# jackdent/cs265-lsm-tree

Hardware: AMD Instinct MI355X
Metric: Bloom build+probe Gkeys/s device-resident; achieved HBM GB/s vs roofline (higher is better)
Workload: dtype int32 keys, u64 hash arithmetic

## Files before the change

cs265-lsm-tree_amd/csrc/bloom_pass1.h:

```cpp
#pragma once

#include "bloom_prims.h"

namespace bloomhip {

namespace {


constexpr int kPrioSort = 0, kPrioScatter = 1, kPrioHash = 2, kPrioYoung = 3;
constexpr int pass1_prio_of(int mode, int level) { return level | mode << 2; }

template <int LAYOUT, int TB>
__device__ __forceinline__ void load_tile_keys(const KeySpan &ks, size_t tile, int tid,
                                               int32_t (&k)[kPartKPT]) {
    static_assert(kPartKPT == 8, "two int4 / four entry pairs per thread");
    const size_t i0 = tile * (size_t)(TB * kPartKPT) + (size_t)kPartKPT * tid;
    const bool full = (tile + 1) * (size_t)(TB * kPartKPT) <= ks.n;
    if constexpr (LAYOUT == KEYS_PACKED) {
        if (full) {
            const int4 *v = reinterpret_cast<const int4 *>(ks.base) + i0 / 4;
            const int4 a = v[0], b = v[1];
            k[0] = a.x; k[1] = a.y; k[2] = a.z; k[3] = a.w;
            k[4] = b.x; k[5] = b.y; k[6] = b.z; k[7] = b.w;
            return;
// ... 2 lines not shown
        if (full) {
            const int4 *v = reinterpret_cast<const int4 *>(ks.base) + i0 / 2;
            const int4 a = v[0], b = v[1], c = v[2], d = v[3];
            k[0] = a.x; k[1] = a.z; k[2] = b.x; k[3] = b.z;
            k[4] = c.x; k[5] = c.z; k[6] = d.x; k[7] = d.z;
            return;
        }
    }
#pragma unroll
    for (int j = 0; j < kPartKPT; j++) {
        const size_t i = i0 + j;
        k[j] = i < ks.n ? load_key<LAYOUT>(ks, i) : 0;
    }
}

__device__ __forceinline__ size_t part_tile(size_t k, size_t ntiles) {
    const size_t base = k * gridDim.x;
    if (base >= ntiles) return ntiles;
    const size_t nr = min((size_t)gridDim.x, ntiles - base);
    return blockIdx.x < nr ? base + xcd_remap(blockIdx.x, (unsigned)nr) : ntiles;
}

template <typename P>
__device__ __forceinline__ uint32_t seg_of(P p, const SegMap &sm) {
    return __umulhi((uint32_t)(p >> sm.shift), sm.magic);
}

constexpr uint32_t kBinShift = 19;

constexpr int kModFast = 0, kModWide = 1, kModP2 = 2, kModLadder = 3, kModLadder0 = 4;
constexpr int kModLadder0R = 5;

template <int MK, int MINW>
__device__ __forceinline__ void bin_entry(uint64_t raw, const ModParams &mp, const SegMap &sm,
                                          uint32_t &b, uint32_t &ent) {
    if constexpr (MK == kModWide) {
        const uint64_t p = mod_wide(raw, mp);
        b = seg_of(p, sm);
        ent = (uint32_t)p & kEntryMask;
    } else if constexpr (MK == kModLadder) {
        const uint32_t xl = (uint32_t)raw;
        const uint32_t a = mod_p2_hi(raw, mp);
        b = __builtin_amdgcn_ubfe(xl, sm.shift, sm.lad_u);
        const uint32_t ehi =
            (a << sm.lad_hb) + __builtin_amdgcn_ubfe(xl, sm.scaled_shift, sm.lad_hb);
        ent = (ehi << sm.shift) | __builtin_amdgcn_ubfe(xl, 0, sm.shift);
    } else if constexpr (MK == kModLadder0) {
        const uint32_t xl = (uint32_t)raw;
        if constexpr (MINW >= 6) {
            const uint32_t lo = __builtin_amdgcn_ubfe(xl, 0, sm.shift);
            b = __builtin_amdgcn_ubfe(xl, sm.shift, sm.lad_u);
            ent = lshl_or_s(mod_p2_hi(raw, mp), sm.shift, lo);
        } else {
            const uint32_t a = mod_p2_hi(raw, mp);
            b = __builtin_amdgcn_ubfe(xl, sm.shift, sm.lad_u);
            ent = (a << sm.shift) | __builtin_amdgcn_ubfe(xl, 0, sm.shift);
        }
    } else if constexpr (MK == kModLadder0R) {
        const uint32_t xl = (uint32_t)raw;
        if constexpr (MINW >= 6) {
            const uint32_t lo = __builtin_amdgcn_ubfe(xl, 0, sm.shift);
            b = __builtin_amdgcn_ubfe(xl, sm.shift, sm.lad_u);
            ent = lshl_or_s(mod_p2_hi24(raw, mp), sm.shift, lo);
        } else {
            const uint32_t a = mod_p2_hi24(raw, mp);
            b = __builtin_amdgcn_ubfe(xl, sm.shift, sm.lad_u);
            ent = (a << sm.shift) | __builtin_amdgcn_ubfe(xl, 0, sm.shift);
        }
    } else if constexpr (MK == kModP2) {
        const uint32_t xl = (uint32_t)raw;
        const uint32_t r = mod_p2_hi(raw, mp);
        const uint32_t q = (r << sm.p2_hi_shift) |
                           __builtin_amdgcn_ubfe(xl, sm.shift, sm.p2_hi_shift);
        b = __umulhi(q, sm.magic);
        ent = xl & kEntryMask;
    } else {
        const uint32_t ru = mod_fast_scaled(raw, mp);
        b = __umulhi(ru >> sm.scaled_shift, sm.magic);
        ent = __builtin_amdgcn_ubfe(ru, mp.l, kEntryBits);
    }
}

template <int LAYOUT, bool SLOTS, bool COLS, int TB, int MK, int MAXB = 0, int MINW = 4,
          int ABL = 0, bool NT = false, bool DEFER = false, int PRIO = 0>
__global__ void __launch_bounds__(TB, MINW) k_part_bin(KeySpan ks, ModParams mp,
                                                       uint64_t *__restrict__ pos_out,
                                                       uint32_t *__restrict__ runs, SegMap sm,
                                                       size_t ntiles, uint16_t *__restrict__ slots) {
    constexpr int kTileKeys = TB * kPartKPT;
    constexpr int kTilePos = 3 * kTileKeys;
    constexpr int kMaxB = MAXB ? MAXB : TB >= 1024 ? (int)kPartMaxBinsBig : (int)kPartMaxBins;
    constexpr int kScanPer = (kMaxB + 1 + TB - 1) / TB;
    static_assert(4 * kTilePos <= (1 << 17) && kTilePos < (1 << 16) &&
                      ((uint64_t)(kMaxB - 1) << kBinShift) < (1ull << 32),
                  "packed rank fields (bin nbins, never incremented, may wrap to 0)");
    constexpr int kPrioLevel = PRIO & 3, kPrioMode = PRIO >> 2;
    static_assert(PRIO == 0 || (kPrioLevel > 0 && kPrioMode <= kPrioYoung), "PRIO = level | mode << 2");
    constexpr bool kFlips = PRIO != 0 && kPrioMode != kPrioYoung;
    constexpr int kPrioAtHist = !kFlips ? -1 : kPrioMode == kPrioHash ? kPrioLevel : 0;
    constexpr int kPrioAtRank = !kFlips || kPrioMode == kPrioScatter ? -1 : kPrioMode == kPrioSort ? kPrioLevel : 0;
    constexpr int kPrioAtScan = kFlips && kPrioMode == kPrioScatter ? kPrioLevel : -1;
    __shared__ __attribute__((aligned(16))) uint32_t s_sorted[kTilePos];
    __shared__ uint32_t s_hist[kMaxB + 1];
    __shared__ uint32_t s_wsum[TB / 64];

    const int tid = threadIdx.x;
    const int lane = tid & 63, wave = tid >> 6;
    const int nb = (int)sm.nbins;
    const int per = (nb + 1 + TB - 1) / TB;
    int32_t kcur[kPartKPT], knext[kPartKPT];

    constexpr int kVecs = kTileKeys / 2;
    constexpr int kStores = kVecs / TB;
    static_assert(kStores * TB == kVecs && kStores * 2 == kPartKPT, "whole vectors per thread");
    auto pack_store = [&](auto full_c, int r, size_t tile, int tile_keys) {
        constexpr bool FULL = decltype(full_c)::value;
        uint4 *dst = reinterpret_cast<uint4 *>(pos_out + tile * (size_t)kTileKeys) + r * TB + tid;
        const uint2 *src = reinterpret_cast<const uint2 *>(s_sorted + 6 * (r * TB + tid));
        const uint2 a = src[0], b = src[1], c = src[2];
        uint32_t e[6] = {a.x, a.y, b.x, b.y, c.x, c.y};
        if constexpr (!FULL) {
#pragma unroll
            for (int q = 0; q < 6; q++) e[q] = 6 * (r * TB + tid) + q < 3 * tile_keys ? e[q] & kEntryMask : 0u;
        }
        const uint4 v = pack_entries6(e);
        if constexpr (ABL == 0) {
            if constexpr (NT) nt_store16(dst, v);
            else *dst = v;
        } else {
            if (v.x == 0xFFFFFFFFu && v.y == 0xFFFFFFFFu) *dst = v;
        }
    };
    constexpr bool kPacks = ABL == 0 || ABL == 5;

    auto do_tile = [&](auto full_c, auto prev_c, size_t tile, size_t next, size_t prev) {
        constexpr bool FULL = decltype(full_c)::value;
        constexpr bool PREV = decltype(prev_c)::value && kPacks;
        const size_t tile0 = tile * kTileKeys;
        const int tile_keys = FULL ? (int)kTileKeys : (int)min((size_t)kTileKeys, ks.n - tile0);
        auto live = [&](int j) { return FULL || kPartKPT * tid + j < tile_keys; };
#pragma clang loop unroll(disable) vectorize(disable)
        for (int b = tid; b <= nb; b += TB) s_hist[b] = (uint32_t)b << kBinShift;
        lds_barrier_prio<kPrioAtHist>();

        uint32_t br[kPartKPT * 3];
        uint32_t ent[kPartKPT * 3];
#pragma unroll
        for (int j = 0; j < kPartKPT; j++) {
            if constexpr (PREV) {
                if (j & 1) pack_store(BoolC<true>{}, j / 2, prev, kTileKeys);
            }
            if (live(j)) {
                const int32_t k = kcur[j];
#pragma unroll
                for (int h = 0; h < 3; h++) {
                    const uint64_t raw = h == 0 ? raw_hash1(k) : h == 1 ? raw_hash2(k) : raw_hash3(k);
                    uint32_t b, e;
                    bin_entry<MK, MINW>(raw, mp, sm, b, e);
                    ent[3 * j + h] = e;
                    if constexpr (ABL == 1) br[3 * j + h] = b;
                    else br[3 * j + h] = atomicAdd(&s_hist[b], 4u);
                }
            } else {
#pragma unroll
                for (int h = 0; h < 3; h++) br[3 * j + h] = ent[3 * j + h] = 0;
            }
        }
        lds_barrier_prio<kPrioAtRank>();
        auto consume = [&]() {
            uint32_t x = 0;
#pragma unroll
            for (int q = 0; q < 3 * kPartKPT; q++) x ^= br[q] + ent[q];
            if (x == 0x9E3779B9u) reinterpret_cast<uint32_t *>(pos_out)[tile * kTileKeys + tid] = x;
        };
        if constexpr (ABL == 1 || ABL == 2) {
            if (next < ntiles) load_tile_keys<LAYOUT, TB>(ks, next, tid, knext);
            consume();
            return;
        }

        const bool scan_wave = wave * 64 * per <= nb;
        uint32_t local[kScanPer];
        uint32_t tsum = 0, incl = 0;
        if (scan_wave) {
#pragma unroll
            for (int q = 0; q < kScanPer; q++) {
                const int b = tid * per + q;
                local[q] = (q < per && b <= nb) ? s_hist[b] - ((uint32_t)b << kBinShift) : 0u;
                tsum += local[q];
            }
            incl = wave_incl_scan(tsum);
            if (lane == 63) s_wsum[wave] = incl;
        }
        lds_barrier();
        if (scan_wave) {
            uint32_t run = incl - tsum;
            for (int w = 0; w < wave; w++) run += s_wsum[w];
#pragma unroll
            for (int q = 0; q < kScanPer; q++) {
                const int b = tid * per + q;
                if (q < per && b <= nb) {
                    s_hist[b] = run - ((uint32_t)b << kBinShift);
                    const uint32_t pk = (run >> 2) | (((run + local[q]) >> 2) << 16);
                    if (b < nb) {
                        if constexpr (COLS) runs[(size_t)b * ntiles + tile] = pk;
                        else runs[tile * (size_t)nb + b] = pk;
                    }
                    run += local[q];
                }
            }
        }
        lds_barrier_prio<kPrioAtScan>();
        if (next < ntiles) load_tile_keys<LAYOUT, TB>(ks, next, tid, knext);
        if constexpr (ABL == 3) {
            consume();
            return;
        }

        const char *hist_b = reinterpret_cast<const char *>(s_hist);
        char *sorted_b = reinterpret_cast<char *>(s_sorted);
#pragma unroll
        for (int h = 0; h < 3; h++) {
            uint32_t slot[kPartKPT];
#pragma unroll
            for (int j = 0; j < kPartKPT; j++)
                slot[j] = *reinterpret_cast<const uint32_t *>(hist_b + (br[3 * j + h] >> 17)) +
                          br[3 * j + h];
#pragma unroll
            for (int j = 0; j < kPartKPT; j++)
                if (live(j)) *reinterpret_cast<uint32_t *>(sorted_b + slot[j]) = ent[3 * j + h];
            if constexpr (SLOTS) {
                uint16_t *sl = slots + (tile * 3 + h) * kTileKeys + kPartKPT * tid;
                if (FULL) {
                    uint32_t w[kPartKPT / 2];
#pragma unroll
                    for (int q = 0; q < kPartKPT / 2; q++)
                        w[q] = lshl_or(slot[2 * q + 1], 14, slot[2 * q] >> 2);
                    typedef uint32_t v4u __attribute__((ext_vector_type(4)));
                    const v4u wv = {w[0], w[1], w[2], w[3]};
                    __builtin_nontemporal_store(wv, reinterpret_cast<v4u *>(sl));
                } else {
#pragma unroll
                    for (int j = 0; j < kPartKPT; j++)
                        if (live(j)) sl[j] = (uint16_t)(slot[j] >> 2);
                }
            }
        }
        lds_barrier();
        if constexpr (ABL == 4) {
            if ((s_sorted[tid] ^ br[0]) == 0x9E3779B9u)
                reinterpret_cast<uint32_t *>(pos_out)[tile * kTileKeys + tid] = br[0];
            return;
        }
        if constexpr (!DEFER) {
#pragma unroll
            for (int r = 0; r < kStores; r++) pack_store(full_c, r, tile, tile_keys);
        }
    };
    auto write_out = [&](auto full_c, size_t tile) {
        if constexpr (DEFER && kPacks) {
            const int tile_keys = (int)min((size_t)kTileKeys, ks.n - tile * kTileKeys);
#pragma unroll
            for (int r = 0; r < kStores; r++) pack_store(full_c, r, tile, tile_keys);
        }
    };

    const size_t nfull = ks.n / kTileKeys;
    size_t tile = part_tile(0, ntiles);
    if (tile >= ntiles) return;
    if constexpr (PRIO != 0 && kPrioMode == kPrioYoung) {
        if (__builtin_amdgcn_readfirstlane(threadIdx.x) >= TB / 2) __builtin_amdgcn_s_setprio(kPrioLevel);
    }
    load_tile_keys<LAYOUT, TB>(ks, tile, tid, kcur);
    if constexpr (!DEFER) {
        for (size_t round = 0; tile < nfull; round++) {
            const size_t next = part_tile(round + 1, ntiles);
            do_tile(BoolC<true>{}, BoolC<false>{}, tile, next, tile);
#pragma unroll
            for (int j = 0; j < kPartKPT; j++) kcur[j] = knext[j];
            tile = next;
        }
        if (tile < ntiles) do_tile(BoolC<false>{}, BoolC<false>{}, tile, ntiles, tile);
    } else if (tile >= nfull) {
        do_tile(BoolC<false>{}, BoolC<false>{}, tile, ntiles, tile);
        write_out(BoolC<false>{}, tile);
    } else {
        size_t prev = tile;
        {
            const size_t next = part_tile(1, ntiles);
            do_tile(BoolC<true>{}, BoolC<false>{}, tile, next, tile);
#pragma unroll
            for (int j = 0; j < kPartKPT; j++) kcur[j] = knext[j];
            tile = next;
        }
        for (size_t round = 1; tile < nfull; round++) {
            const size_t next = part_tile(round + 1, ntiles);
            do_tile(BoolC<true>{}, BoolC<true>{}, tile, next, prev);
#pragma unroll
            for (int j = 0; j < kPartKPT; j++) kcur[j] = knext[j];
            prev = tile;
            tile = next;
        }
        if (tile < ntiles) {
            do_tile(BoolC<false>{}, BoolC<true>{}, tile, ntiles, prev);
            write_out(BoolC<false>{}, tile);
        } else {
            write_out(BoolC<true>{}, prev);
        }
    }
}

constexpr uint32_t kBinShift2 = 20;
constexpr int kSuperBlock = 1024;

template <int LAYOUT>
__device__ __forceinline__ void load_half_keys(const KeySpan &ks, size_t tile, int half, int tid,
                                               int32_t (&k)[kPartKPT]) {
    constexpr size_t kHalf = (size_t)kSuperBlock * kPartKPT;
    const size_t i0 = tile * kSuperTileKeys + half * kHalf + (size_t)kPartKPT * tid;
    const bool full = tile * kSuperTileKeys + (half + 1) * kHalf <= ks.n;
    if constexpr (LAYOUT == KEYS_PACKED) {
        if (full) {
            const int4 *v = reinterpret_cast<const int4 *>(ks.base) + i0 / 4;
            const int4 a = v[0], b = v[1];
            k[0] = a.x; k[1] = a.y; k[2] = a.z; k[3] = a.w;
            k[4] = b.x; k[5] = b.y; k[6] = b.z; k[7] = b.w;
            return;
        }
    } else if constexpr (LAYOUT == KEYS_ENTRY) {
        if (full) {
            const int4 *v = reinterpret_cast<const int4 *>(ks.base) + i0 / 2;
            const int4 a = v[0], b = v[1], c = v[2], d = v[3];
            k[0] = a.x; k[1] = a.z; k[2] = b.x; k[3] = b.z;
            k[4] = c.x; k[5] = c.z; k[6] = d.x; k[7] = d.z;
            return;
        }
    }
#pragma unroll
    for (int j = 0; j < kPartKPT; j++) {
        const size_t i = i0 + j;
        k[j] = i < ks.n ? load_key<LAYOUT>(ks, i) : 0;
    }
}

template <int LAYOUT, bool COLS, int MK, int MAXB, bool SLOTS = false>
__global__ void __launch_bounds__(kSuperBlock, 4) k_part_bin2(KeySpan ks, ModParams mp,
                                                              uint64_t *__restrict__ pos_out,
                                                              uint32_t *__restrict__ runs, SegMap sm,
                                                              size_t ntiles, uint16_t *__restrict__ slots) {
    constexpr int TB = kSuperBlock;
    constexpr int kHalfKeys = TB * kPartKPT;
    constexpr int kTileKeys = 2 * kHalfKeys;
    constexpr int kTilePos = 3 * kTileKeys;
    constexpr int kPhasePos = kTilePos / 2;
    constexpr uint32_t kPhaseBytes = 4u * kPhasePos;
    constexpr int kScanPer = (MAXB + 1 + TB - 1) / TB;
    constexpr int kPer = 3 * kPartKPT;
// ... 150 lines not shown
#pragma unroll
        for (int ph = 0; ph < 2; ph++) {
            const uint32_t base = ph * kPhaseBytes;
            uint2 w[kPartKPT];
#pragma unroll
            for (int j = 0; j < kPartKPT; j++) w[j] = stash[j * TB + tid];
#pragma unroll
            for (int j = 0; j < kPartKPT; j++) {
#pragma unroll
                for (int h = 0; h < 3; h++) {
                    const uint32_t la = brA[3 * j + h] - base;
                    if (la < kPhaseBytes) {
                        const uint32_t e = h == 0 ? w[j].x & kEntryMask
                                         : h == 1 ? __builtin_amdgcn_alignbit(w[j].y, w[j].x, 21) & kEntryMask
                                                  : w[j].y >> 10;
                        *reinterpret_cast<uint32_t *>(img_b + la) = e;
                    }
                }
            }
#pragma unroll
            for (int j = 0; j < kPartKPT; j++) {
#pragma unroll
                for (int h = 0; h < 3; h++) {
                    const uint32_t lb = brB[3 * j + h] - base;
                    if (lb < kPhaseBytes) {
                        const uint32_t lo = eB[2 * j], hi = eB[2 * j + 1];
                        const uint32_t e = h == 0 ? lo & kEntryMask
                                         : h == 1 ? __builtin_amdgcn_alignbit(hi, lo, 21) & kEntryMask
                                                  : hi >> 10;
                        *reinterpret_cast<uint32_t *>(img_b + lb) = e;
                    }
                }
            }
            lds_barrier();
#pragma unroll
            for (int r = 0; r < kStores; r++) {
                const uint2 *src = reinterpret_cast<const uint2 *>(img + 6 * (r * TB + tid));
                const uint2 a = src[0], b = src[1], c = src[2];
                uint32_t e[6] = {a.x, a.y, b.x, b.y, c.x, c.y};
                if constexpr (!FULL) {
#pragma unroll
                    for (int z = 0; z < 6; z++) e[z] &= kEntryMask;
                }
                dst[ph * kVecs + r * TB + tid] = pack_entries6(e);
            }
            if (ph == 0) lds_barrier();
        }
    };

    const size_t nfull = ks.n / kTileKeys;
    size_t tile = part_tile(0, ntiles);
    if (tile < ntiles) load_half_keys<LAYOUT>(ks, tile, 0, (int)threadIdx.x, kA);
    size_t round = 0;
    for (; tile < nfull; round++) {
        const size_t next = part_tile(round + 1, ntiles);
        do_tile(BoolC<true>{}, tile, next);
        tile = next;
    }
    if (tile < ntiles) do_tile(BoolC<false>{}, tile, ntiles);
}

constexpr size_t kColumnTableMaxBytes = 16u << 20;
constexpr int kTransposeTile = 64;
constexpr int kTransposeBlock = 256;

}

hipError_t launch_runs_transpose(const PartitionWorkspace &ws, hipStream_t stream);
bool runs_as_columns(const PartitionWorkspace &ws);

struct Pass1Kernel {
    bool super;
    int threads;
    int layout;
    bool slots;
    bool cols;
    int mk;
    int maxb;
    int wgs_per_cu;
    bool nt;
    bool defer;
    unsigned grid;
    int prio;
};
using Pass1Launch = bool(const Pass1Kernel &p, const KeySpan &ks, const ModParams &mp,
                         const PartitionWorkspace &ws, const SegMap &sm, uint16_t *slots,
                         hipStream_t stream);
Pass1Launch launch_bin_build512, launch_bin_build1024, launch_bin_probe512, launch_bin_probe1024,
    launch_bin_super, launch_bin_super_probe;

namespace {

constexpr int pass1_max_bins(bool super, int threads) {
    return super ? (int)kSuperMaxBins : threads >= 1024 ? (int)kPartMaxBinsBig : (int)kPartMaxBins;
}

constexpr bool pass1_takes_kind(bool super, bool slots, int mk) {
    if (super) return mk == kModP2 || mk == kModFast;
    return mk >= 0 && !(slots && (mk == kModLadder0 || mk == kModLadder0R));
}

constexpr int pass1_capacity(int threads, int layout, int mk, size_t nbins) {
    const int cap = pass1_max_bins(false, threads);
    if (layout == KEYS_STRIDED || mk == kModWide) return cap;
    if (threads >= 1024) return nbins <= 1023 ? 1023 : nbins <= 2047 ? 2047 : nbins <= 4095 ? 4095 : cap;
    return nbins <= 511 ? 511 : cap;
}

constexpr int pass1_wgs_per_cu(int threads, bool slots, int maxb) {
    return threads >= 1024 ? 1 : (!slots && maxb > 0 && maxb <= 511) ? 3 : 2;
}
constexpr int pass1_min_waves(int threads, int wgs) { return wgs * threads / 256; }
inline unsigned pass1_grid(size_t ntiles, int ncu, int wgs) {
    const size_t g = (size_t)ncu * wgs;
    return (unsigned)(ntiles < g ? ntiles : g);
}

constexpr bool pass1_defer(int threads, bool slots) { return threads >= 1024 && !slots; }

constexpr int pass1_prio(int threads, bool slots, int wgs_per_cu) {
    return threads == 512 && !slots && wgs_per_cu == 3 ? pass1_prio_of(kPrioHash, 1) : 0;
}

constexpr bool pass1_may_nt(int threads, bool slots, int maxb) {
    return !slots && threads >= 1024 && maxb == 1023;
}

inline bool p2_pass1(const ModParams &mp, const SegMap &sm) {
    return mp.fast && mp.p2 && mp.p2t >= kEntryBits && sm.shift <= mp.p2t && mp.p2t - sm.shift < 32;
}

inline int pass1_plan(const ModParams &mp, const PartitionWorkspace &ws, bool slots, SegMap *out) {
    SegMap sm = seg_map_of(ws);
    const bool wide = !mp.fast;
    if (!wide) {
        sm.scaled_shift = sm.shift + mp.l;
        if (sm.scaled_shift > 31) {
            sm.scaled_shift = 0;
            sm.magic = 0;
        }
    }
    int mk;
    if (ws.lad_u) {
        if (!mp.fast || !mp.p2 || sm.shift + sm.lad_u + sm.lad_hb != mp.p2t) return -1;
        sm.scaled_shift = sm.shift + sm.lad_u;
        mk = sm.lad_hb == 0 && !slots ? (ladder0_relabel(mp, ws) ? kModLadder0R : kModLadder0) : kModLadder;
    } else if (wide) {
        mk = kModWide;
    } else if (p2_pass1(mp, sm)) {
        sm.p2_hi_shift = mp.p2t - sm.shift;
        mk = kModP2;
    } else {
        mk = kModFast;
    }
    *out = sm;
    return mk;
}

inline bool choose_pass1_kernel(const KeySpan &ks, const ModParams &mp, const PartitionWorkspace &ws,
                                bool slots, int ncu, Pass1Kernel *out, SegMap *sm) {
    Pass1Kernel p{};
    p.super = tile_keys_of(ws) == kSuperTileKeys;
    p.threads = p.super ? kSuperBlock : tile_keys_of(ws) == 2 * kPartTileKeys ? 1024 : 512;
    p.slots = slots;
    if (ws.nbins > (size_t)pass1_max_bins(p.super, p.threads)) return false;
    p.mk = pass1_plan(mp, ws, slots, sm);
    if (p.mk < 0 || !pass1_takes_kind(p.super, slots, p.mk)) return false;
    p.layout = ks.layout == KEYS_PACKED ? KEYS_PACKED
               : ks.layout == KEYS_ENTRY && (reinterpret_cast<uintptr_t>(ks.base) & 15) == 0 ? KEYS_ENTRY
                                                                                               : KEYS_STRIDED;
    p.maxb = p.super ? (int)kSuperMaxBins : pass1_capacity(p.threads, p.layout, p.mk, ws.nbins);
    p.wgs_per_cu = p.super ? 1 : pass1_wgs_per_cu(p.threads, slots, p.maxb);
    p.defer = !p.super && pass1_defer(p.threads, slots);
    p.nt = !p.super && pass1_may_nt(p.threads, slots, p.maxb) &&
           ws.ntiles * (uint64_t)(p.threads * kPartKPT) * 8 > kInfinityCacheBytes;
    p.prio = p.super ? 0 : pass1_prio(p.threads, slots, p.wgs_per_cu);
    p.cols = runs_as_columns(ws);
    p.grid = pass1_grid(ws.ntiles, ncu, p.wgs_per_cu);
    *out = p;
    return true;
}

template <bool SLOTS, int TB>
bool launch_pass1_tile(const Pass1Kernel &p, const KeySpan &ks, const ModParams &mp,
                       const PartitionWorkspace &ws, const SegMap &sm, uint16_t *slots,
                       hipStream_t stream) {
    constexpr bool kDefer = pass1_defer(TB, SLOTS);
    if (p.super || p.threads != TB || p.slots != SLOTS || p.defer != kDefer) return false;
    uint32_t *runs = p.cols ? ws.run_starts : ws.run_rows;
    return on_value<kModFast, kModWide, kModP2, kModLadder, kModLadder0, kModLadder0R>(p.mk, [&](auto mk_c) {
        return on_value<KEYS_PACKED, KEYS_ENTRY, KEYS_STRIDED>(p.layout, [&](auto layout_c) {
            return on_value<511, 1023, 2047, 4095, pass1_max_bins(false, TB)>(p.maxb, [&](auto maxb_c) {
                constexpr int MK = decltype(mk_c)::value, L = decltype(layout_c)::value;
                constexpr int MAXB = decltype(maxb_c)::value;
                constexpr bool kHeld = pass1_takes_kind(false, SLOTS, MK) && pass1_capacity(TB, L, MK, MAXB) == MAXB;
                if constexpr (kHeld) {
                    constexpr int kWgs = pass1_wgs_per_cu(TB, SLOTS, MAXB);
                    constexpr int kMinW = pass1_min_waves(TB, kWgs);
                    constexpr bool kMayNT = pass1_may_nt(TB, SLOTS, MAXB);
                    constexpr int kPrio = pass1_prio(TB, SLOTS, kWgs);
                    if (p.wgs_per_cu != kWgs || (p.nt && !kMayNT) || p.prio != kPrio) return false;
                    auto go = [&](auto cols_c, auto nt_c) {
                        k_part_bin<L, SLOTS, decltype(cols_c)::value, TB, MK, MAXB, kMinW, 0,
                                   decltype(nt_c)::value, kDefer, kPrio>
                            <<<p.grid, TB, 0, stream>>>(ks, mp, ws.pos, runs, sm, ws.ntiles, slots);
                    };
                    if constexpr (kMayNT) {
                        if (p.nt) {
                            p.cols ? go(BoolC<true>{}, BoolC<true>{}) : go(BoolC<false>{}, BoolC<true>{});
                            return true;
                        }
                    }
                    p.cols ? go(BoolC<true>{}, BoolC<false>{}) : go(BoolC<false>{}, BoolC<false>{});
                    return true;
                } else {
                    return false;
                }
            });
        });
    });
}

template <bool SLOTS>
bool launch_pass1_super(const Pass1Kernel &p, const KeySpan &ks, const ModParams &mp,
                        const PartitionWorkspace &ws, const SegMap &sm, uint16_t *slots,
                        hipStream_t stream) {
    if (!p.super || p.slots != SLOTS) return false;
    uint32_t *runs = p.cols ? ws.run_starts : ws.run_rows;
    return on_value<kModP2, kModFast>(p.mk, [&](auto mk_c) {
        return on_value<KEYS_PACKED, KEYS_ENTRY, KEYS_STRIDED>(p.layout, [&](auto layout_c) {
            auto go = [&](auto cols_c) {
                k_part_bin2<decltype(layout_c)::value, decltype(cols_c)::value, decltype(mk_c)::value,
                            (int)kSuperMaxBins, SLOTS>
                    <<<p.grid, kSuperBlock, 0, stream>>>(ks, mp, ws.pos, runs, sm, ws.ntiles, slots);
            };
            p.cols ? go(BoolC<true>{}) : go(BoolC<false>{});
            return true;
        });
    });
}

template <bool SLOTS>
hipError_t launch_bin(const KeySpan &ks, const ModParams &mp, const PartitionWorkspace &ws,
                      uint16_t *slots, hipStream_t stream) {
    Pass1Kernel p{};
    SegMap sm{};
    if ((SLOTS && !slots) || !choose_pass1_kernel(ks, mp, ws, SLOTS, device_cu_count(), &p, &sm))
        return hipErrorInvalidValue;
    Pass1Launch *unit;
    if constexpr (SLOTS)
        unit = p.super ? launch_bin_super_probe : p.threads >= 1024 ? launch_bin_probe1024 : launch_bin_probe512;
    else
        unit = p.super ? launch_bin_super : p.threads >= 1024 ? launch_bin_build1024 : launch_bin_build512;
    if (!unit(p, ks, mp, ws, sm, SLOTS ? slots : nullptr, stream)) return hipErrorInvalidValue;
    const hipError_t e = hipGetLastError();
    if (e != hipSuccess || p.cols) return e;
    return launch_runs_transpose(ws, stream);
}

}

}
```

cs265-lsm-tree_amd/csrc/ubench.hip:

```cpp
#include <hip/hip_runtime.h>
#include <stdint.h>
#include <stdio.h>

#include <algorithm>
#include <numeric>

#include "bloom_combine.h"
#include "bloom_pass1.h"
#include "bloom_pass2.h"
#include "bloom_merge.h"

using namespace bloomhip;

namespace {

__device__ __forceinline__ uint32_t xorshift(uint32_t &s) {
    s ^= s << 13;
    s ^= s >> 17;
    s ^= s << 5;
    return s;
}

template <int SCOPE>
__global__ void ub_atomic_or(uint32_t *words, uint32_t nwords, int iters) {
// ... 241 lines not shown
    return 0;
}

namespace {
StackTable ladder0_table(const ModParams &mp, const PartitionWorkspace &ws) {
    StackTable st{};
    st.lad.s = ws.lad_s;
    st.lad.u = ws.lad_u;
    st.lad.d = mp.p2d;
    st.lad.t[0] = mp.p2t;
    st.lad.rinv = ladder0_relabel(mp, ws) ? ladder0_inv(mp) : 0u;
    return st;
}

bool build_plan(size_t n, uint64_t m, int ncu, PartitionWorkspace *ws, int *mode) {
    if (!plan_build(m, ncu, ws)) return false;
    if (!ws->tile_keys) ws->tile_keys = choose_tile_keys(ws->nbins);
    ws->ntiles = (n + ws->tile_keys - 1) / ws->tile_keys;
    *mode = ws->lad_u ? kApplyBuildL : kApplyBuild;
    return true;
}
}

extern "C" int ubench_walk_choice(size_t n, int nf, const uint64_t *ms, int cu_count, int *out7) {
    PartitionWorkspace ws{};
    int mode = 0;
    if (nf == 1) {
        if (!build_plan(n, ms[0], cu_count, &ws, &mode)) return -34;
    } else {
        StackTable st{};
        uint64_t mmax = 0, g = 0, mmin = ~0ull;
        for (int j = 0; j < nf; j++) {
            mmax = std::max(mmax, ms[j]);
            mmin = std::min(mmin, ms[j]);
            g = std::gcd(g, ms[j]);
        }
        const bool ladder = plan_ladder(ms, nf, cu_count, &st, &ws);
        if (!ladder && !plan_stack(mmax, g, mmin, nf, cu_count, &ws)) return -34;
        if (!ws.tile_keys) ws.tile_keys = choose_tile_keys(ws.nbins);
        ws.ntiles = (n + ws.tile_keys - 1) / ws.tile_keys;
        mode = ladder ? kApplyLadder : kApplyStack;
    }
    const ApplyWalk w = choose_apply_walk(mode, ws.tile_keys, ws.nbins, ws.ntiles);
    const int out[7] = {mode, (int)ws.tile_keys, (int)ws.nbins, w.g, w.chains, w.vecs, (int)w.redir};
    std::copy(out, out + 7, out7);
    return 0;
}

namespace {
int pass1_choice_of(size_t n, uint64_t m, int slots, size_t stride, int cu_count, Pass1Kernel *out) {
    PartitionWorkspace ws{};
    int mode = 0;
    if (slots) {
        if (!plan_segments(m, cu_count, &ws)) return -34;
        ws.tile_keys = choose_tile_keys(ws.nbins);
        ws.ntiles = (n + ws.tile_keys - 1) / ws.tile_keys;
    } else if (!build_plan(n, m, cu_count, &ws, &mode)) {
        return -34;
    }
    const KeySpan ks{nullptr, n, stride, stride == 4 ? KEYS_PACKED : stride == 8 ? KEYS_ENTRY : KEYS_STRIDED};
    SegMap sm{};
    if (!choose_pass1_kernel(ks, make_mod_params(m), ws, slots != 0, cu_count, out, &sm)) return -22;
    return 0;
}
}

extern "C" int ubench_pass1_choice(size_t n, uint64_t m, int slots, size_t stride, int cu_count,
                                   int *out11) {
    Pass1Kernel p{};
    const int rc = pass1_choice_of(n, m, slots, stride, cu_count, &p);
    if (rc) return rc;
    const int out[11] = {p.super, p.threads, p.layout, p.slots, p.cols, p.mk, p.maxb, p.wgs_per_cu,
                         p.nt, p.defer, (int)p.grid};
    std::copy(out, out + 11, out11);
    return 0;
}

extern "C" int ubench_pass1_prio(size_t n, uint64_t m, int slots, size_t stride, int cu_count,
                                 int *prio_out) {
    Pass1Kernel p{};
    const int rc = pass1_choice_of(n, m, slots, stride, cu_count, &p);
    if (rc) return rc;
    *prio_out = p.prio;
    return 0;
}

extern "C" int ubench_part_walk(int chains, int vecs, int redir, const void *keys, size_t n,
                                uint64_t m, uint64_t *pos, uint32_t *runs, uint32_t *words,
                                void *stream, size_t pos_cap, size_t runs_cap) {
    hipStream_t s = reinterpret_cast<hipStream_t>(stream);
    const KeySpan ks{reinterpret_cast<const char *>(keys), n, 4, KEYS_PACKED};
    const ModParams mp = make_mod_params(m);
    PartitionWorkspace ws{};
    int mode = 0;
    if (n == 0) return -22;
    if (!build_plan(n, m, device_cu_count(), &ws, &mode)) return -34;
    if (ws.ntiles * ws.tile_keys > pos_cap || 2 * ws.ntiles * (ws.nbins + 1) > runs_cap) return -28;
    ws.pos = pos;
    ws.run_rows = runs;
    ws.run_starts = runs + ws.ntiles * (ws.nbins + 1);
    hipError_t e = launch_part_bin(ks, mp, ws, s);
    if (e != hipSuccess) {
        fprintf(stderr, "ubench_part_walk: pass 1: %s\n", hipGetErrorString(e));
        return -5;
    }
    const StackTable st = mode == kApplyBuildL ? ladder0_table(mp, ws) : StackTable{};
    const uint64_t nw32 = ((mp.m + 63) / 64) * 2;
    const ApplyWalk w{4, chains, vecs, redir != 0};
    e = hipErrorInvalidValue;
#define UB_ON(MODE, TK, C, V, R)                                                                  \
    if (mode == MODE && ws.tile_keys == TK && w == ApplyWalk{4, C, V, R})                         \
        e = launch_apply_g<MODE, 4, TK, 1, C, V, R>(ws, mp.m, words, nw32, 0, nullptr, st, s);
#define UB_WALKS(MODE, TK) \
    UB_ON(MODE, TK, 1, 1, false) UB_ON(MODE, TK, 1, 1, true) UB_ON(MODE, TK, 1, 2, true) UB_ON(MODE, TK, 2, 2, true)
    UB_WALKS(kApplyBuildL, 4096) UB_WALKS(kApplyBuildL, 8192)
    UB_WALKS(kApplyBuild, 4096) UB_WALKS(kApplyBuild, 8192) UB_WALKS(kApplyBuild, 16384)
#undef UB_WALKS
#undef UB_ON
    if (e != hipSuccess) fprintf(stderr, "ubench_part_walk: pass 2: %s\n", hipGetErrorString(e));
    return e == hipSuccess ? 0 : e == hipErrorInvalidValue ? -22 : -5;
}

extern "C" int ubench_part(int variant, const void *keys, size_t n, uint64_t m, uint64_t *pos,
                           uint32_t *runs, uint32_t *words, void *stream, size_t pos_cap,
                           size_t runs_cap) {
    hipStream_t s = reinterpret_cast<hipStream_t>(stream);
    const KeySpan ks{reinterpret_cast<const char *>(keys), n, 4, KEYS_PACKED};
    const ModParams mp = make_mod_params(m);
    PartitionWorkspace ws{};
    const bool seg = variant == 20 || variant == 21;
    if (!(seg ? plan_segments(m, device_cu_count(), &ws) : plan_build(m, device_cu_count(), &ws)))
        return -34;
    if (!ws.tile_keys) ws.tile_keys = choose_tile_keys(ws.nbins);
    ws.ntiles = (n + ws.tile_keys - 1) / ws.tile_keys;
    if (ws.ntiles * ws.tile_keys > pos_cap || 2 * ws.ntiles * (ws.nbins + 1) > runs_cap) return -28;
    ws.pos = pos;
    ws.run_rows = runs;
    ws.run_starts = runs + ws.ntiles * (ws.nbins + 1);
    hipError_t e = hipSuccess;
    switch (variant) {
        case 0: case 20: e = launch_part_bin(ks, mp, ws, s); break;
        case 1: case 21: e = launch_part_apply(mp, words, ws, 0, s); break;
#define UB_P2(V, TB, MAXB, NWG)                                                                   \
    case V: {                                                                                    \
        if (ws.nbins > MAXB || ws.tile_keys != TB * kPartKPT || !mp.p2) return -22;             \
        SegMap sm = seg_map_of(ws);                                                              \
        sm.p2_hi_shift = mp.p2t - sm.shift;                                                      \
        k_part_bin<KEYS_PACKED, false, true, TB, kModP2, MAXB, pass1_min_waves(TB, NWG)>         \
            <<<pass1_grid(ws.ntiles, device_cu_count(), NWG), TB, 0, s>>>(                       \
                ks, mp, ws.pos, ws.run_starts, sm, ws.ntiles, nullptr);                          \
        e = hipGetLastError();                                                                   \
        break;                                                                                   \
    }
        UB_P2(5001, 512, 511, 2) UB_P2(5003, 512, 511, pass1_wgs_per_cu(512, false, 511))
#undef UB_P2
        case 2503: case 2507: case 2522: case 2523: {
            if (ws.lad_u || tile_keys_of(ws) != kSuperTileKeys) return -22;
            const uint64_t nw32 = ((mp.m + 63) / 64) * 2;
            constexpr int TK = (int)kSuperTileKeys;
#define UB_WALK(V, G, C, NV, R)                                                                   \
    if (variant == V)                                                                             \
        e = launch_apply_g<kApplyBuild, G, TK, 1, C, NV, R>(ws, mp.m, words, nw32, 0, nullptr, StackTable{}, s);
            UB_WALK(2503, 4, 1, 2, true) UB_WALK(2507, 4, 2, 2, true) UB_WALK(2522, 4, 1, 1, true)
            UB_WALK(2523, 2, 1, 2, true)
#undef UB_WALK
            break;
        }
        case 2401: case 2413: case 2417: {
            if (!ws.lad_u || ws.lad_hb != 0 || !mp.p2) return -22;
            const StackTable st = ladder0_table(mp, ws);
            const uint64_t nw32 = ((mp.m + 63) / 64) * 2;
            const size_t tk = tile_keys_of(ws);
            if (tk != 4096 && tk != 8192) return -22;
#define UB_WALK(V, C, NV, R)                                                                      \
    if (variant == V)                                                                             \
        e = tk == 4096 ? launch_apply_g<kApplyBuildL, 4, 4096, 1, C, NV, R>(ws, mp.m, words, nw32, 0, nullptr, st, s) \
                       : launch_apply_g<kApplyBuildL, 4, 8192, 1, C, NV, R>(ws, mp.m, words, nw32, 0, nullptr, st, s);
            UB_WALK(2401, 1, 1, false) UB_WALK(2413, 1, 2, true) UB_WALK(2417, 2, 2, true)
#undef UB_WALK
            break;
        }
#define UB_ABL(A, D)                                                                              \
    case 5100 + 20 * D + A: {                                                                    \
        SegMap sm{};                                                                             \
        if (pass1_plan(mp, ws, false, &sm) != kModLadder0R || ws.tile_keys != 4096 ||           \
            ws.nbins > 511 || !runs_as_columns(ws))                                              \
            return -22;                                                                          \
        constexpr int kWgs = pass1_wgs_per_cu(512, false, 511);                                  \
        k_part_bin<KEYS_PACKED, false, true, 512, kModLadder0R, 511, pass1_min_waves(512, kWgs), A, false, D != 0> \
            <<<pass1_grid(ws.ntiles, device_cu_count(), kWgs), 512, 0, s>>>(                     \
                ks, mp, ws.pos, ws.run_starts, sm, ws.ntiles, nullptr);                          \
        e = hipGetLastError();                                                                   \
        break;                                                                                   \
    }
        UB_ABL(0, 0) UB_ABL(1, 0) UB_ABL(2, 0) UB_ABL(3, 0) UB_ABL(4, 0) UB_ABL(5, 0)
        UB_ABL(0, 1) UB_ABL(5, 1)
#undef UB_ABL
#define UB_PRIO(P, A)                                                                             \
    case 5200 + 10 * P + A: {                                                                    \
        SegMap sm{};                                                                             \
        if (pass1_plan(mp, ws, false, &sm) != kModLadder0R || ws.tile_keys != 4096 ||           \
            ws.nbins > 511 || !runs_as_columns(ws))                                              \
            return -22;                                                                          \
        constexpr int kWgs = pass1_wgs_per_cu(512, false, 511);                                  \
        k_part_bin<KEYS_PACKED, false, true, 512, kModLadder0R, 511, pass1_min_waves(512, kWgs), A, false, false, P> \
            <<<pass1_grid(ws.ntiles, device_cu_count(), kWgs), 512, 0, s>>>(                     \
                ks, mp, ws.pos, ws.run_starts, sm, ws.ntiles, nullptr);                          \
        e = hipGetLastError();                                                                   \
        break;                                                                                   \
    }
#define UB_PRIO_LADDER(P) UB_PRIO(P, 0) UB_PRIO(P, 3) UB_PRIO(P, 4) UB_PRIO(P, 5)
        UB_PRIO_LADDER(pass1_prio_of(kPrioSort, 1)) UB_PRIO_LADDER(pass1_prio_of(kPrioSort, 2))
        UB_PRIO_LADDER(pass1_prio_of(kPrioSort, 3)) UB_PRIO_LADDER(pass1_prio_of(kPrioScatter, 1))
        UB_PRIO_LADDER(pass1_prio_of(kPrioHash, 1)) UB_PRIO(pass1_prio_of(kPrioHash, 2), 0)
        UB_PRIO(pass1_prio_of(kPrioHash, 3), 0) UB_PRIO(pass1_prio_of(kPrioYoung, 1), 0)
#undef UB_PRIO_LADDER
#undef UB_PRIO
        case 5413: {
            SegMap sm{};
            const int mk = pass1_plan(mp, ws, false, &sm);
            constexpr int kP = pass1_prio_of(kPrioYoung, 1);
            if (ws.tile_keys != 8192 || ws.nbins > 1023 || !runs_as_columns(ws)) return -22;
            const unsigned grid = pass1_grid(ws.ntiles, device_cu_count(), 1);
            const bool nt = ws.ntiles * (uint64_t)8192 * 8 > kInfinityCacheBytes;
            if (mk == kModLadder0R && nt)
                k_part_bin<KEYS_PACKED, false, true, 1024, kModLadder0R, 1023, 4, 0, true, true, kP>
                    <<<grid, 1024, 0, s>>>(ks, mp, ws.pos, ws.run_starts, sm, ws.ntiles, nullptr);
            else if (mk == kModFast && !nt)
                k_part_bin<KEYS_PACKED, false, true, 1024, kModFast, 1023, 4, 0, false, true, kP>
                    <<<grid, 1024, 0, s>>>(ks, mp, ws.pos, ws.run_starts, sm, ws.ntiles, nullptr);
            else
                return -22;
            e = hipGetLastError();
            break;
        }
        default: return -22;
    }
    return e == hipSuccess ? 0 : -5;
}

namespace {
bool ub_stack_plan(int nf, const uint64_t *ms, uint64_t *mmax, PartitionWorkspace *ws) {
    uint64_t g = 0;
    *mmax = 0;
    for (int j = 0; j < nf; j++) {
        *mmax = ms[j] > *mmax ? ms[j] : *mmax;
        g = g == 0 || ms[j] < g ? ms[j] : g;
    }
    return plan_stack(*mmax, g, g, nf, device_cu_count(), ws);
}
}

extern "C" int ubench_stack_geometry(int nf, const uint64_t *ms, uint64_t *nbins_out,
                                     uint64_t *seg_bits_out) {
    uint64_t mmax = 0;
    PartitionWorkspace ws{};
    if (!ub_stack_plan(nf, ms, &mmax, &ws)) return -34;
    *nbins_out = ws.nbins;
    *seg_bits_out = ws.seg_bits;
    return 0;
}

extern "C" int ubench_stack(int variant, const void *keys, size_t n, int nf, const uint64_t *ms,
                            void *const *words, uint64_t *pos, uint32_t *runs, uint8_t *res,
                            uint16_t *slots, uint64_t *out, void *stream) {
    hipStream_t s = reinterpret_cast<hipStream_t>(stream);
    const KeySpan ks{reinterpret_cast<const char *>(keys), n, 4, KEYS_PACKED};
    uint64_t mmax = 0;
    PartitionWorkspace ws{};
    if (!ub_stack_plan(nf, ms, &mmax, &ws)) return -34;
    ws.tile_keys = choose_tile_keys(ws.nbins);
    ws.ntiles = (n + ws.tile_keys - 1) / ws.tile_keys;
    ws.pos = pos;
    ws.run_rows = runs;
    ws.run_starts = runs + ws.ntiles * (ws.nbins + 1);
    StackTable st{};
    st.nf = nf;
    for (int j = 0; j < nf; j++) {
        st.words[j] = reinterpret_cast<const uint32_t *>(words[j]);
        st.mwords[j] = (uint32_t)(ms[j] / 32);
        st.row[j] = j;
    }
    const ModParams mp = make_mod_params(mmax);
    const size_t nw = (n + 63) / 64;
    hipError_t e = hipSuccess;
    switch (variant) {
        case 0: e = launch_probe_stacked(ks, mp, st, ws, res, slots, out, nw, s); break;
        case 1: e = launch_bin<true>(ks, mp, ws, slots, s); break;
        case 2: e = launch_apply_stack(ws, mmax, res, st, s); break;
        case 5: e = launch_combine(ws, res, slots, n, out, nw, st, s); break;
        default: return -22;
    }
    return e == hipSuccess ? 0 : -5;
}

extern "C" int ubench_ladder(int variant, int tile_keys, const void *keys, size_t n, int nf,
                             const uint64_t *ms, void *const *words, uint64_t *pos,
                             uint32_t *runs, uint8_t *res, uint16_t *slots, uint64_t *out,
                             void *stream) {
    hipStream_t s = reinterpret_cast<hipStream_t>(stream);
// ... 201 lines not shown
```

Baseline: 206.3.

## Software-pipeline pass1 partition with double-buffered histograms across tiles

Adds a PIPE variant of the partition kernel that keeps two histograms in LDS. Each tile's hashing and ranking overlap the scatter and packed store of the previous tile, and one of the per-tile barriers is removed. It is enabled by default for 512-thread, 3-WG/CU ladder-mod configurations. It costs extra LDS for the second histogram and more registers held live across iterations, which may affect occupancy.

```diff
diff --git a/cs265-lsm-tree_amd/csrc/bloom_pass1.h b/cs265-lsm-tree_amd/csrc/bloom_pass1.h
--- a/cs265-lsm-tree_amd/csrc/bloom_pass1.h
+++ b/cs265-lsm-tree_amd/csrc/bloom_pass1.h
@@ -108,7 +108,7 @@
 }
 
 template <int LAYOUT, bool SLOTS, bool COLS, int TB, int MK, int MAXB = 0, int MINW = 4,
-          int ABL = 0, bool NT = false, bool DEFER = false, int PRIO = 0>
+          int ABL = 0, bool NT = false, bool DEFER = false, int PRIO = 0, int PIPE = 0>
 __global__ void __launch_bounds__(TB, MINW) k_part_bin(KeySpan ks, ModParams mp,
                                                        uint64_t *__restrict__ pos_out,
                                                        uint32_t *__restrict__ runs, SegMap sm,
@@ -127,7 +127,7 @@
     constexpr int kPrioAtRank = !kFlips || kPrioMode == kPrioScatter ? -1 : kPrioMode == kPrioSort ? kPrioLevel : 0;
     constexpr int kPrioAtScan = kFlips && kPrioMode == kPrioScatter ? kPrioLevel : -1;
     __shared__ __attribute__((aligned(16))) uint32_t s_sorted[kTilePos];
-    __shared__ uint32_t s_hist[kMaxB + 1];
+    __shared__ uint32_t s_hist[(PIPE ? 2 : 1) * (kMaxB + 1)];
     __shared__ uint32_t s_wsum[TB / 64];
 
     const int tid = threadIdx.x;
@@ -159,6 +159,41 @@
     };
     constexpr bool kPacks = ABL == 0 || ABL == 5;
 
+    auto scan_counts = [&](uint32_t hoff, uint32_t (&local)[kScanPer], uint32_t &tsum, uint32_t &incl) {
+        const bool scan_wave = wave * 64 * per <= nb;
+        tsum = incl = 0;
+        if (scan_wave) {
+#pragma unroll
+            for (int q = 0; q < kScanPer; q++) {
+                const int b = tid * per + q;
+                local[q] = (q < per && b <= nb) ? s_hist[hoff + b] - ((hoff + b) << kBinShift) : 0u;
+                tsum += local[q];
+            }
+            incl = wave_incl_scan(tsum);
+            if (lane == 63) s_wsum[wave] = incl;
+        }
+    };
+    auto scan_offsets = [&](uint32_t hoff, size_t tile, const uint32_t (&local)[kScanPer], uint32_t tsum,
+                            uint32_t incl) {
+        if (wave * 64 * per <= nb) {
+            uint32_t run = incl - tsum;
+            for (int w = 0; w < wave; w++) run += s_wsum[w];
+#pragma unroll
+            for (int q = 0; q < kScanPer; q++) {
+                const int b = tid * per + q;
+                if (q < per && b <= nb) {
+                    s_hist[hoff + b] = run - ((hoff + b) << kBinShift);
+                    const uint32_t pk = (run >> 2) | (((run + local[q]) >> 2) << 16);
+                    if (b < nb) {
+                        if constexpr (COLS) runs[(size_t)b * ntiles + tile] = pk;
+                        else runs[tile * (size_t)nb + b] = pk;
+                    }
+                    run += local[q];
+                }
+            }
+        }
+    };
+
     auto do_tile = [&](auto full_c, auto prev_c, size_t tile, size_t next, size_t prev) {
         constexpr bool FULL = decltype(full_c)::value;
         constexpr bool PREV = decltype(prev_c)::value && kPacks;
@@ -205,37 +240,11 @@
             return;
         }
 
-        const bool scan_wave = wave * 64 * per <= nb;
         uint32_t local[kScanPer];
-        uint32_t tsum = 0, incl = 0;
-        if (scan_wave) {
-#pragma unroll
-            for (int q = 0; q < kScanPer; q++) {
-                const int b = tid * per + q;
-                local[q] = (q < per && b <= nb) ? s_hist[b] - ((uint32_t)b << kBinShift) : 0u;
-                tsum += local[q];
-            }
-            incl = wave_incl_scan(tsum);
-            if (lane == 63) s_wsum[wave] = incl;
-        }
+        uint32_t tsum, incl;
+        scan_counts(0u, local, tsum, incl);
         lds_barrier();
-        if (scan_wave) {
-            uint32_t run = incl - tsum;
-            for (int w = 0; w < wave; w++) run += s_wsum[w];
-#pragma unroll
-            for (int q = 0; q < kScanPer; q++) {
-                const int b = tid * per + q;
-                if (q < per && b <= nb) {
-                    s_hist[b] = run - ((uint32_t)b << kBinShift);
-                    const uint32_t pk = (run >> 2) | (((run + local[q]) >> 2) << 16);
-                    if (b < nb) {
-                        if constexpr (COLS) runs[(size_t)b * ntiles + tile] = pk;
-                        else runs[tile * (size_t)nb + b] = pk;
-                    }
-                    run += local[q];
-                }
-            }
-        }
+        scan_offsets(0u, tile, local, tsum, incl);
         lds_barrier_prio<kPrioAtScan>();
         if (next < ntiles) load_tile_keys<LAYOUT, TB>(ks, next, tid, knext);
         if constexpr (ABL == 3) {
@@ -298,7 +307,122 @@
         if (__builtin_amdgcn_readfirstlane(threadIdx.x) >= TB / 2) __builtin_amdgcn_s_setprio(kPrioLevel);
     }
     load_tile_keys<LAYOUT, TB>(ks, tile, tid, kcur);
-    if constexpr (!DEFER) {
+    if constexpr (PIPE != 0) {
+        static_assert(!DEFER && !SLOTS && (PRIO == 0 || kPrioMode == kPrioHash),
+                      "PIPE: a build's loop; phase A holds the hash phase's priority");
+        constexpr uint32_t kHist = kMaxB + 1;
+        static_assert(((uint64_t)(2 * kHist - 1) << kBinShift) < (1ull << 32), "both histograms' bins in the rank field");
+        uint32_t br[kPartKPT * 3];
+        uint32_t ent[kPartKPT * 3];
+        constexpr bool kScatters = ABL == 0 || ABL >= 4;
+        auto scatter_key = [&](int j, bool alive) {
+            const char *hist_b = reinterpret_cast<const char *>(s_hist);
+            char *sorted_b = reinterpret_cast<char *>(s_sorted);
+            uint32_t slot[3];
+#pragma unroll
+            for (int h = 0; h < 3; h++)
+                slot[h] = *reinterpret_cast<const uint32_t *>(hist_b + (br[3 * j + h] >> 17)) + br[3 * j + h];
+            if (alive) {
+#pragma unroll
+                for (int h = 0; h < 3; h++) *reinterpret_cast<uint32_t *>(sorted_b + slot[h]) = ent[3 * j + h];
+            }
+        };
+        auto consume = [&](size_t tile) {
+            uint32_t x = 0;
+#pragma unroll
+            for (int q = 0; q < 3 * kPartKPT; q++) x ^= br[q] + ent[q];
+            if (x == 0x9E3779B9u) reinterpret_cast<uint32_t *>(pos_out)[tile * kTileKeys + tid] = x;
+        };
+        auto consume_image = [&](size_t tile) {
+            if ((s_sorted[tid] ^ br[0]) == 0x9E3779B9u)
+                reinterpret_cast<uint32_t *>(pos_out)[tile * kTileKeys + tid] = br[0];
+        };
+        auto pipe_tile = [&](auto full_c, auto prev_c, size_t tile, size_t next, size_t prev, uint32_t hoff) {
+            constexpr bool FULL = decltype(full_c)::value, PREV = decltype(prev_c)::value;
+            const int tile_keys = FULL ? (int)kTileKeys : (int)min((size_t)kTileKeys, ks.n - tile * kTileKeys);
+            auto live = [&](int j) { return FULL || kPartKPT * tid + j < tile_keys; };
+#pragma unroll
+            for (int j = 0; j < kPartKPT; j++) {
+                if constexpr (PREV && kScatters) scatter_key(j, true);
+                if (live(j)) {
+                    const int32_t k = kcur[j];
+#pragma unroll
+                    for (int h = 0; h < 3; h++) {
+                        const uint64_t raw = h == 0 ? raw_hash1(k) : h == 1 ? raw_hash2(k) : raw_hash3(k);
+                        uint32_t b, e;
+                        bin_entry<MK, MINW>(raw, mp, sm, b, e);
+                        ent[3 * j + h] = e;
+                        if constexpr (ABL == 1) br[3 * j + h] = b;
+                        else br[3 * j + h] = atomicAdd(&s_hist[hoff + b], 4u);
+                    }
+                } else {
+#pragma unroll
+                    for (int h = 0; h < 3; h++) br[3 * j + h] = ent[3 * j + h] = 0;
+                }
+            }
+            lds_barrier_prio<kPrioAtRank>();
+            uint32_t local[kScanPer];
+            uint32_t tsum, incl;
+            if constexpr (ABL == 0 || ABL >= 3) scan_counts(hoff, local, tsum, incl);
+            const uint32_t other = kHist - hoff;
+#pragma clang loop unroll(disable) vectorize(disable)
+            for (int b = tid; b <= nb; b += TB) s_hist[other + b] = (other + b) << kBinShift;
+            if constexpr (ABL == 0 || ABL >= 3) {
+                lds_barrier();
+                scan_offsets(hoff, tile, local, tsum, incl);
+            }
+            if (next < ntiles) load_tile_keys<LAYOUT, TB>(ks, next, tid, kcur);
+            if constexpr (ABL >= 1 && ABL <= 3) consume(tile);
+            if constexpr (PREV) {
+                if constexpr (ABL == 4) consume_image(prev);
+                if constexpr (kPacks) {
+#pragma unroll
+                    for (int r = 0; r < kStores; r++) pack_store(BoolC<true>{}, r, prev, kTileKeys);
+                }
+            }
+            lds_barrier_prio<kPrioAtHist>();
+        };
+        auto pipe_last = [&](auto full_c, size_t tile) {
+            constexpr bool FULL = decltype(full_c)::value;
+            const int tile_keys = FULL ? (int)kTileKeys : (int)min((size_t)kTileKeys, ks.n - tile * kTileKeys);
+            if constexpr (kScatters) {
+#pragma unroll
+                for (int j = 0; j < kPartKPT; j++) scatter_key(j, FULL || kPartKPT * tid + j < tile_keys);
+                lds_barrier_prio<kPrioAtRank>();
+                if constexpr (ABL == 4) consume_image(tile);
+            }
+            if constexpr (kPacks) {
+#pragma unroll
+                for (int r = 0; r < kStores; r++) pack_store(full_c, r, tile, tile_keys);
+            }
+        };
+
+#pragma clang loop unroll(disable) vectorize(disable)
+        for (int b = tid; b <= nb; b += TB) s_hist[b] = (uint32_t)b << kBinShift;
+        lds_barrier_prio<kPrioAtHist>();
+        if (tile >= nfull) {
+            pipe_tile(BoolC<false>{}, BoolC<false>{}, tile, ntiles, tile, 0u);
+            pipe_last(BoolC<false>{}, tile);
+            return;
+        }
+        size_t prev = tile, next = part_tile(1, ntiles);
+        pipe_tile(BoolC<true>{}, BoolC<false>{}, tile, next, tile, 0u);
+        tile = next;
+        uint32_t hoff = kHist;
+        for (size_t round = 2; tile < nfull; round++) {
+            next = part_tile(round, ntiles);
+            pipe_tile(BoolC<true>{}, BoolC<true>{}, tile, next, prev, hoff);
+            prev = tile;
+            tile = next;
+            hoff = kHist - hoff;
+        }
+        if (tile < ntiles) {
+            pipe_tile(BoolC<false>{}, BoolC<true>{}, tile, ntiles, prev, hoff);
+            pipe_last(BoolC<false>{}, tile);
+        } else {
+            pipe_last(BoolC<true>{}, prev);
+        }
+    } else if constexpr (!DEFER) {
         for (size_t round = 0; tile < nfull; round++) {
             const size_t next = part_tile(round + 1, ntiles);
             do_tile(BoolC<true>{}, BoolC<false>{}, tile, next, tile);
@@ -615,6 +739,7 @@
     bool defer;
     unsigned grid;
     int prio;
+    int pipe;
 };
 using Pass1Launch = bool(const Pass1Kernel &p, const KeySpan &ks, const ModParams &mp,
                          const PartitionWorkspace &ws, const SegMap &sm, uint16_t *slots,
@@ -653,6 +778,10 @@
 
 constexpr int pass1_prio(int threads, bool slots, int wgs_per_cu) {
     return threads == 512 && !slots && wgs_per_cu == 3 ? pass1_prio_of(kPrioHash, 1) : 0;
+}
+
+constexpr int pass1_pipe(int threads, bool slots, int wgs_per_cu, int mk) {
+    return threads == 512 && !slots && wgs_per_cu == 3 && (mk == kModLadder0 || mk == kModLadder0R) ? 1 : 0;
 }
 
 constexpr bool pass1_may_nt(int threads, bool slots, int maxb) {
@@ -708,6 +837,7 @@
     p.nt = !p.super && pass1_may_nt(p.threads, slots, p.maxb) &&
            ws.ntiles * (uint64_t)(p.threads * kPartKPT) * 8 > kInfinityCacheBytes;
     p.prio = p.super ? 0 : pass1_prio(p.threads, slots, p.wgs_per_cu);
+    p.pipe = p.super ? 0 : pass1_pipe(p.threads, slots, p.wgs_per_cu, p.mk);
     p.cols = runs_as_columns(ws);
     p.grid = pass1_grid(ws.ntiles, ncu, p.wgs_per_cu);
     *out = p;
@@ -732,10 +862,11 @@
                     constexpr int kMinW = pass1_min_waves(TB, kWgs);
                     constexpr bool kMayNT = pass1_may_nt(TB, SLOTS, MAXB);
                     constexpr int kPrio = pass1_prio(TB, SLOTS, kWgs);
-                    if (p.wgs_per_cu != kWgs || (p.nt && !kMayNT) || p.prio != kPrio) return false;
+                    constexpr int kPipe = pass1_pipe(TB, SLOTS, kWgs, MK);
+                    if (p.wgs_per_cu != kWgs || (p.nt && !kMayNT) || p.prio != kPrio || p.pipe != kPipe) return false;
                     auto go = [&](auto cols_c, auto nt_c) {
                         k_part_bin<L, SLOTS, decltype(cols_c)::value, TB, MK, MAXB, kMinW, 0,
-                                   decltype(nt_c)::value, kDefer, kPrio>
+                                   decltype(nt_c)::value, kDefer, kPrio, kPipe>
                             <<<p.grid, TB, 0, stream>>>(ks, mp, ws.pos, runs, sm, ws.ntiles, slots);
                     };
                     if constexpr (kMayNT) {
diff --git a/cs265-lsm-tree_amd/csrc/ubench.hip b/cs265-lsm-tree_amd/csrc/ubench.hip
--- a/cs265-lsm-tree_amd/csrc/ubench.hip
+++ b/cs265-lsm-tree_amd/csrc/ubench.hip
@@ -347,6 +347,15 @@
     const int rc = pass1_choice_of(n, m, slots, stride, cu_count, &p);
     if (rc) return rc;
     *prio_out = p.prio;
+    return 0;
+}
+
+extern "C" int ubench_pass1_pipe(size_t n, uint64_t m, int slots, size_t stride, int cu_count,
+                                 int *pipe_out) {
+    Pass1Kernel p{};
+    const int rc = pass1_choice_of(n, m, slots, stride, cu_count, &p);
+    if (rc) return rc;
+    *pipe_out = p.pipe;
     return 0;
 }
 
@@ -481,6 +490,22 @@
         UB_PRIO(pass1_prio_of(kPrioHash, 3), 0) UB_PRIO(pass1_prio_of(kPrioYoung, 1), 0)
 #undef UB_PRIO_LADDER
 #undef UB_PRIO
+#define UB_PIPE(A)                                                                                \
+    case 5500 + A: {                                                                             \
+        SegMap sm{};                                                                             \
+        if (pass1_plan(mp, ws, false, &sm) != kModLadder0R || ws.tile_keys != 4096 ||           \
+            ws.nbins > 511 || !runs_as_columns(ws))                                              \
+            return -22;                                                                          \
+        constexpr int kWgs = pass1_wgs_per_cu(512, false, 511);                                  \
+        k_part_bin<KEYS_PACKED, false, true, 512, kModLadder0R, 511, pass1_min_waves(512, kWgs), A, false, false, \
+                   pass1_prio_of(kPrioHash, 1), 1>                                               \
+            <<<pass1_grid(ws.ntiles, device_cu_count(), kWgs), 512, 0, s>>>(                     \
+                ks, mp, ws.pos, ws.run_starts, sm, ws.ntiles, nullptr);                          \
+        e = hipGetLastError();                                                                   \
+        break;                                                                                   \
+    }
+        UB_PIPE(0) UB_PIPE(1) UB_PIPE(2) UB_PIPE(3) UB_PIPE(4) UB_PIPE(5)
+#undef UB_PIPE
         case 5413: {
             SegMap sm{};
             const int mk = pass1_plan(mp, ws, false, &sm);
```

After: 214.5 (median of 6 runs). 4.0% higher.
